# calclavia/tal-asrd

Measured on AMD Instinct MI355X. Metric: audio frames/sec (16 kHz, 10 ms hop) end-to-end log-mel -> TDS encoder -> diarization head, higher is better.
Workload: dtype f32 (dense layers: 3 x f16 MFMA hi/lo split, f32 accumulate); 1 GPU; 1 x 3600 s 16 kHz clip per GPU, each a whole-episode B=1 call (BASELINE.json configs[2]; SDModel path of tal/baseline/reconcile.py:76-85: log-mel -> TDS 80-800-1120-1440 -> 128-d feat + argmax over 6008 speakers); weights=synthetic deterministic, audio_resident_in_hbm=True

## Files before the change

tal_asrd_amd/csrc/gemm_common.h:

```cpp
#pragma once
#include "common.h"

namespace tal {

constexpr int BK = 32;

template <int MODE, int NSUB>
__device__ __forceinline__ void gemm_epilogue(const GemmArgs& g, const f32x16 (&acc)[NSUB], float* lds, float* Y,
                                              const float* bias, const float* res, int64_t m0, int n0, int lane,
                                              int w, int wm, int wn) {
    const int64_t M = g.M;
    const int N = g.N;
    const int colb = lane & 31;
    const int rowb = 4 * (lane >> 5);
    const float alpha = g.alpha;
    const f32x4 zero4 = {0.f, 0.f, 0.f, 0.f};
    float amax = 0.f;
    constexpr int CW = 32 * NSUB;
    if (MODE == 4) {
        float bcol[NSUB];
#pragma unroll
        for (int j = 0; j < NSUB; ++j) {
            const int col = n0 + (wn * NSUB + j) * 32 + colb;
            bcol[j] = (bias && col < N) ? bias[col] : 0.f;
        }
        const int pcol = (n0 / CW) + wn;
#pragma unroll
        for (int e = 0; e < 16; ++e) {
            float best = -INFINITY;
            int bi = 0x7fffffff;
#pragma unroll
            for (int j = 0; j < NSUB; ++j) {
                const int col = n0 + (wn * NSUB + j) * 32 + colb;
                const float v = acc[j][e] + bcol[j];
                if (col < N && v > best) {
                    best = v;
                    bi = col;
                }
            }
#pragma unroll
            for (int off = 16; off > 0; off >>= 1) {
                const float ov = __shfl_xor(best, off, 64);
                const int oi = __shfl_xor(bi, off, 64);
                if (ov > best || (ov == best && oi < bi)) {
                    best = ov;
                    bi = oi;
                }
            }
            const int64_t row = m0 + wm * 32 + rowb + (e & 3) + 8 * (e >> 2);
            if (colb == 0 && row < M) {
                g.part_val[row * g.part_ld + pcol] = best;
                g.part_idx[row * g.part_ld + pcol] = bi;
            }
        }
        return;
    }
    const bool vec_ok = (g.ldy % 4 == 0) && (MODE != 2 || g.ldres % 4 == 0) &&
                        ((reinterpret_cast<uintptr_t>(Y) & 15) == 0) &&
                        (MODE != 2 || (reinterpret_cast<uintptr_t>(res) & 15) == 0);
    if (vec_ok) {
        float* stage = lds + w * (16 * CW);
        const int n_base = n0 + wn * CW;
        const bool cols_full = n_base + CW <= N;
        const bool buf_ok = g.ldy < (1 << 21) && (MODE != 2 || g.ldres < (1 << 21));
        auto uptr = [](const float* p) {
            const uint64_t v = reinterpret_cast<uint64_t>(p);
            const uint32_t lo = __builtin_amdgcn_readfirstlane((uint32_t)v), hi = __builtin_amdgcn_readfirstlane((uint32_t)(v >> 32));
            return reinterpret_cast<void*>(((uint64_t)hi << 32) | lo);
        };
        __amdgpu_buffer_rsrc_t rs_y[2], rs_res[2];
#pragma unroll
        for (int half = 0; half < 2; ++half) {
            const int64_t row0 = m0 + wm * 32 + half * 16;
            const int rows_valid = (int)(M - row0 < 0 ? 0 : (M - row0 > 16 ? 16 : M - row0));
            const int ext_y = rows_valid > 0 ? (int)(((rows_valid - 1) * g.ldy + CW) * 4) : 0;
            const int ext_r = rows_valid > 0 && MODE == 2 ? (int)(((rows_valid - 1) * g.ldres + CW) * 4) : 0;
            rs_y[half] = __builtin_amdgcn_make_buffer_rsrc(uptr(Y + row0 * g.ldy + n_base), 0, __builtin_amdgcn_readfirstlane(ext_y), 0x00020000);
            rs_res[half] = __builtin_amdgcn_make_buffer_rsrc(uptr(MODE == 2 ? res + row0 * g.ldres + n_base : Y), 0,
                                                             __builtin_amdgcn_readfirstlane(ext_r), 0x00020000);
        }
        __amdgpu_buffer_rsrc_t rs_bias = __builtin_amdgcn_make_buffer_rsrc(uptr(bias ? bias + n_base : Y), 0, CW * 4, 0x00020000);
#pragma unroll
        for (int half = 0; half < 2; ++half) {
#pragma unroll
            for (int j = 0; j < NSUB; ++j)
#pragma unroll
                for (int e8 = 0; e8 < 8; ++e8) {
                    const int e = half * 8 + e8;
                    const int r = rowb + (e8 & 3) + 8 * (e8 >> 2);
                    stage[r * CW + j * 32 + colb] = acc[j][e];
                }
            if (cols_full && buf_ok) {
                typedef unsigned u32x4 __attribute__((ext_vector_type(4)));
                int r = lane / (CW / 4), c4 = lane - r * (CW / 4);
                int offy[2 * NSUB], offr[2 * NSUB], offb[2 * NSUB], ldsv[2 * NSUB];
                f32x4 rv[2 * NSUB], bv[2 * NSUB];
#pragma unroll
                for (int t = 0; t < 2 * NSUB; ++t) {
                    offy[t] = (r * (int)g.ldy + c4 * 4) * 4;
                    offr[t] = (r * (int)g.ldres + c4 * 4) * 4;
                    offb[t] = c4 * 16;
                    ldsv[t] = r * CW + c4 * 4;
                    c4 += 64 - CW / 4;
                    r += 1;
                    if (c4 >= CW / 4) {
                        c4 -= CW / 4;
                        r += 1;
                    }
                }
                typedef unsigned u32x2r __attribute__((ext_vector_type(2)));
                u32x2r rh[2 * NSUB], rl[2 * NSUB];
#pragma unroll
                for (int t = 0; t < 2 * NSUB; ++t) {
                    if (MODE == 2 && g.res_split) {
                        const int cw = offb[t] >> 2;
                        const int so = offr[t] - offb[t] + (cw >> 5) * 128 + (cw & 31) * 2;
                        rh[t] = __builtin_amdgcn_raw_buffer_load_b64(rs_res[half], so, 0, 0);
                        rl[t] = __builtin_amdgcn_raw_buffer_load_b64(rs_res[half], so + 64, 0, 0);
                    } else if (MODE == 2)
                        rv[t] = __builtin_bit_cast(f32x4, __builtin_amdgcn_raw_buffer_load_b128(rs_res[half], offr[t], 0, 0));
                    bv[t] = bias ? __builtin_bit_cast(f32x4, __builtin_amdgcn_raw_buffer_load_b128(rs_bias, offb[t], 0, 0)) : zero4;
                }
#pragma unroll
                for (int t = 0; t < 2 * NSUB; ++t) {
// ... 38 lines not shown
                if (g.out_split && half == 1) note_range(amax, g.range_flag);
                continue;
            }
#pragma unroll
            for (int t = 0; t < 2 * NSUB; ++t) {
                const int i = lane + 64 * t;
                const int r = i / (CW / 4);
                const int c = (i - r * (CW / 4)) * 4;
                const int64_t row = m0 + wm * 32 + half * 16 + r;
                const int col = n_base + c;
                if (row < M && col < N) {
                    f32x4 v = *reinterpret_cast<const f32x4*>(&stage[r * CW + c]);
                    if (col + 3 < N) {
                        if (bias) v += *reinterpret_cast<const f32x4*>(bias + col);
                        if (MODE == 1) {
                            v.x = fmaxf(v.x, 0.f); v.y = fmaxf(v.y, 0.f); v.z = fmaxf(v.z, 0.f); v.w = fmaxf(v.w, 0.f);
                        }
                        if (MODE == 2) v = *reinterpret_cast<const f32x4*>(res + row * g.ldres + col) + alpha * v;
                        if (MODE == 3 && (g.scale_cols == 0 || col < g.scale_cols)) v = alpha * v;
                        *reinterpret_cast<f32x4*>(Y + row * g.ldy + col) = v;
                    } else {
                        for (int q = 0; q < 4 && col + q < N; ++q) {
                            float x = v[q] + (bias ? bias[col + q] : 0.f);
                            if (MODE == 1) x = fmaxf(x, 0.f);
                            if (MODE == 2) x = res[row * g.ldres + col + q] + alpha * x;
                            if (MODE == 3 && (g.scale_cols == 0 || col + q < g.scale_cols)) x = alpha * x;
                            Y[row * g.ldy + col + q] = x;
                        }
                    }
                }
            }
        }
    } else {
#pragma unroll
        for (int j = 0; j < NSUB; ++j) {
            const int col = n0 + (wn * NSUB + j) * 32 + colb;
            if (col >= N) continue;
            const float bv = bias ? bias[col] : 0.f;
#pragma unroll
            for (int e = 0; e < 16; ++e) {
                const int64_t row = m0 + wm * 32 + rowb + (e & 3) + 8 * (e >> 2);
                if (row < M) {
                    float v = acc[j][e] + bv;
                    if (MODE == 1) v = fmaxf(v, 0.f);
                    if (MODE == 2) v = res[row * g.ldres + col] + alpha * v;
                    if (MODE == 3 && (g.scale_cols == 0 || col < g.scale_cols)) v = alpha * v;
                    Y[row * g.ldy + col] = v;
                }
            }
        }
    }
}

template <int MODE, int NSUB>
__device__ __forceinline__ void gemm_epilogue_split(const GemmArgs& g, const f32x16 (&acc)[NSUB], float* lds, float* Y,
                                                    const float* res, int64_t m0, int n0, int lane, int w) {
    static_assert(MODE == 1 || MODE == 2, "relu or residual");
    constexpr int CW = 32 * NSUB;
    typedef unsigned u32x2 __attribute__((ext_vector_type(2)));
    typedef float f32x2 __attribute__((ext_vector_type(2)));
    const int64_t M = g.M;
    const int colb = lane & 31, rowb = 4 * (lane >> 5);
    float* stage = lds + w * (16 * CW);
    auto uptr = [](const float* p) {
        const uint64_t v = reinterpret_cast<uint64_t>(p);
        const uint32_t lo = __builtin_amdgcn_readfirstlane((uint32_t)v), hi = __builtin_amdgcn_readfirstlane((uint32_t)(v >> 32));
        return reinterpret_cast<void*>(((uint64_t)hi << 32) | lo);
    };
    const int lr = lane >> 3, lp = lane & 7;
    const int ldy4 = (int)g.ldy * 4, ldr4 = (int)g.ldres * 4;
    const int vy0 = lr * ldy4 + lp * 8, vy1 = vy0 + 8 * ldy4;
    const int vr0 = lr * ldr4 + lp * 8, vr1 = vr0 + 8 * ldr4;
    const float* sp = stage + lr * CW + lp * 4;
    const float alpha = g.alpha;
    const f32x2 al2 = {alpha, alpha}, s11 = {1.0f / 2048.0f, 1.0f / 2048.0f};
    float amax = 0.f;
#pragma unroll
    for (int half = 0; half < 2; ++half) {
        const int64_t row0 = m0 + w * 32 + half * 16;
        const int rows_valid = (int)(M - row0 < 0 ? 0 : (M - row0 > 16 ? 16 : M - row0));
        const int ext_y = rows_valid > 0 ? (rows_valid - 1) * ldy4 + CW * 4 : 0;
        const int ext_r = rows_valid > 0 && MODE == 2 ? (rows_valid - 1) * ldr4 + CW * 4 : 0;
        __amdgpu_buffer_rsrc_t rs_y = __builtin_amdgcn_make_buffer_rsrc(uptr(Y + row0 * g.ldy + n0), 0, __builtin_amdgcn_readfirstlane(ext_y), 0x00020000);
        __amdgpu_buffer_rsrc_t rs_r = __builtin_amdgcn_make_buffer_rsrc(uptr(MODE == 2 ? res + row0 * g.ldres + n0 : Y), 0,
                                                                      __builtin_amdgcn_readfirstlane(ext_r), 0x00020000);
        u32x2 rh[2 * NSUB], rl[2 * NSUB];
        if (MODE == 2) {
#pragma unroll
            for (int t = 0; t < 2 * NSUB; ++t) {
                const int rg = t / NSUB, b = t % NSUB;
                rh[t] = __builtin_amdgcn_raw_buffer_load_b64(rs_r, (rg ? vr1 : vr0) + b * 128, 0, 0);
                rl[t] = __builtin_amdgcn_raw_buffer_load_b64(rs_r, (rg ? vr1 : vr0) + b * 128 + 64, 0, 0);
            }
        }
#pragma unroll
        for (int j = 0; j < NSUB; ++j)
#pragma unroll
            for (int e8 = 0; e8 < 8; ++e8) {
                const int r = rowb + (e8 & 3) + 8 * (e8 >> 2);
                stage[r * CW + j * 32 + colb] = acc[j][half * 8 + e8];
            }
        f32x4 sv[2 * NSUB];
#pragma unroll
        for (int t = 0; t < 2 * NSUB; ++t) sv[t] = *reinterpret_cast<const f32x4*>(sp + (t / NSUB) * 8 * CW + (t % NSUB) * 32);
#pragma unroll
        for (int t = 0; t < 2 * NSUB; ++t) {
            const int rg = t / NSUB, b = t % NSUB;
            f32x2 va = {sv[t][0], sv[t][1]}, vb = {sv[t][2], sv[t][3]};
            if (MODE == 1) {
                va = __builtin_elementwise_max(va, f32x2{0.f, 0.f});
                vb = __builtin_elementwise_max(vb, f32x2{0.f, 0.f});
            } else {
                const f16x4 h4 = __builtin_bit_cast(f16x4, rh[t]), l4 = __builtin_bit_cast(f16x4, rl[t]);
                const f32x2 ha = {(float)h4[0], (float)h4[1]}, hb = {(float)h4[2], (float)h4[3]};
                const f32x2 la = {(float)l4[0], (float)l4[1]}, lb = {(float)l4[2], (float)l4[3]};
                va = al2 * va + (la * s11 + ha);
                vb = al2 * vb + (lb * s11 + hb);
            }
            amax = __builtin_fmaxf(amax, __builtin_fmaxf(__builtin_fabsf(va[0]), __builtin_fabsf(va[1])));
            amax = __builtin_fmaxf(amax, __builtin_fmaxf(__builtin_fabsf(vb[0]), __builtin_fabsf(vb[1])));
            f16x2p h01, l01, h23, l23;
            split_f16x3_pair(va[0], va[1], h01, l01);
            split_f16x3_pair(vb[0], vb[1], h23, l23);
            const f16x4 hi = {h01[0], h01[1], h23[0], h23[1]}, lo = {l01[0], l01[1], l23[0], l23[1]};
            __builtin_amdgcn_raw_buffer_store_b64(__builtin_bit_cast(u32x2, hi), rs_y, (rg ? vy1 : vy0) + b * 128, 0, 0);
            __builtin_amdgcn_raw_buffer_store_b64(__builtin_bit_cast(u32x2, lo), rs_y, (rg ? vy1 : vy0) + b * 128 + 64, 0, 0);
        }
    }
    note_range(amax, g.range_flag);
}

__device__ __forceinline__ unsigned logical_tile_of(unsigned nb, unsigned bid) {
    const unsigned xcd = bid & 7u, q = nb >> 3, r = nb & 7u;
    return (xcd < r ? xcd * (q + 1) : r * (q + 1) + (xcd - r) * q) + (bid >> 3);
// ... 5 lines not shown
```

tal_asrd_amd/csrc/gemm_f32.hip:

```cpp
#include "gemm_common.h"

namespace tal {

template <int MODE, int NSUB, bool SPLITK, int STAGE, bool F16X3 = false, int EPI = 0>
__global__ __launch_bounds__(256, F16X3 ? 2 : 1) void gemm_glds_kernel(const GemmArgs g) {
    __builtin_amdgcn_s_setprio(3);
    constexpr int BM = 128, BN = 32 * NSUB;
    constexpr int ROWS = BM + BN;
    constexpr int CHUNKS = ROWS / 8;
    constexpr int PER_WAVE = CHUNKS / 4;
    __shared__ __attribute__((aligned(16))) float lds[2 * ROWS * 32];

    const bool is_slice = SPLITK && blockIdx.x >= (unsigned)g.tile_base;
    const unsigned sbid = blockIdx.x - (unsigned)g.tile_base;
    const int slice = is_slice ? (int)(sbid / (unsigned)g.tail_tiles) : 0;
    const unsigned logical = is_slice ? (unsigned)g.tile_base + sbid % (unsigned)g.tail_tiles
                                      : (SPLITK ? logical_tile_of((unsigned)g.tile_base, blockIdx.x) : logical_tile());
    const unsigned tile_m = g.tiles_n == 1 ? logical : __umulhi(logical, g.tiles_n_magic);
    const int64_t m0 = (int64_t)tile_m * BM;
    const int n0 = (int)(logical - tile_m * (unsigned)g.tiles_n) * BN;
    const int64_t M = g.M;
    const int N = g.N, K = g.K;
    const int z1 = EPI ? 0 : (int)blockIdx.y / g.nb2, z2 = EPI ? 0 : (int)blockIdx.y % g.nb2;
    const float* A = g.A + z1 * g.a_s1 + z2 * g.a_s2;
// ... 18 lines not shown
        if (t < 4)
            src[t] = A + (m0 + min(row, a_rows)) * g.lda + srccol;
        else
            src[t] = W + (int64_t)(n0 + min(row - BM, b_rows)) * g.ldw + srccol;
    }
    auto uniform_ptr = [](const float* p) {
        const uint64_t v = reinterpret_cast<uint64_t>(p);
        const uint32_t lo = __builtin_amdgcn_readfirstlane((uint32_t)v), hi = __builtin_amdgcn_readfirstlane((uint32_t)(v >> 32));
        return reinterpret_cast<void*>(((uint64_t)hi << 32) | lo);
    };
    __amdgpu_buffer_rsrc_t rsrc_a = __builtin_amdgcn_make_buffer_rsrc(uniform_ptr(A + m0 * g.lda), 0, 0x7fffffff, 0x00020000);
    __amdgpu_buffer_rsrc_t rsrc_w = __builtin_amdgcn_make_buffer_rsrc(uniform_ptr(W + (int64_t)n0 * g.ldw), 0, 0x7fffffff, 0x00020000);
    int voff[PER_WAVE];
#pragma unroll
    for (int t = 0; t < PER_WAVE; ++t) {
        const int row = 8 * (w + 4 * t) + sub;
        voff[t] = t < 4 ? (int)((min(row, a_rows) * g.lda + srccol) * 4) : (int)((min(row - BM, b_rows) * g.ldw + srccol) * 4);
    }
    auto issue = [&](int kt, int buf) {
#pragma unroll
        for (int t = 0; t < PER_WAVE; ++t) {
            float* dst = lds + buf * (ROWS * 32) + (w + 4 * t) * 256;
            if (STAGE == 2) {
#if defined(__HIP_DEVICE_COMPILE__)
                __builtin_amdgcn_raw_ptr_buffer_load_lds(t < 4 ? rsrc_a : rsrc_w, (__attribute__((address_space(3))) void*)dst, 16,
                                                         voff[t], kt * (BK * 4), 0, 0);
#endif
            } else
                __builtin_amdgcn_global_load_lds((const __attribute__((address_space(1))) void*)(src[t] + kt * BK),
                                                 (__attribute__((address_space(3))) void*)dst, 16, 0, 0);
        }
    };

    f32x16 acc[NSUB];
    f32x16 accx[F16X3 ? NSUB : 1];
#pragma unroll
    for (int j = 0; j < NSUB; ++j) {
        const float b0 = (EPI && bias && !is_slice) ? bias[n0 + j * 32 + (lane & 31)] : 0.f;
#pragma unroll
        for (int e = 0; e < 16; ++e) acc[j][e] = b0;
    }
#pragma unroll
    for (int j = 0; j < (F16X3 ? NSUB : 1); ++j)
#pragma unroll
        for (int e = 0; e < 16; ++e) accx[j][e] = 0.f;

    const int frow = lane & 31;
    const int fsw = (frow >> 1) & 7;
    const int fhalf = lane >> 5;
    const int nk_all = K / BK;
    const int kt0 = is_slice ? (int)((int64_t)slice * nk_all / g.split) : 0;
    const int nk = is_slice ? (int)((int64_t)(slice + 1) * nk_all / g.split) : nk_all;
    issue(kt0, kt0 & 1);
    __builtin_amdgcn_s_setprio(0);
    __builtin_assume(kt0 < nk);
    for (int kt = kt0; kt < nk; ++kt) {
        asm volatile("s_waitcnt vmcnt(0)" ::: "memory");
        __syncthreads();
        if (kt + 1 < nk) issue(kt + 1, (kt + 1) & 1);
        const float* As = lds + (kt & 1) * (ROWS * 32) + (wm * 32 + frow) * 32;
        const float* Bs = lds + (kt & 1) * (ROWS * 32) + (BM + frow) * 32;
        if (F16X3) {
            f16x8 ahi[2], alo[2], bhi[3], blo[3];
            auto slh = [&](int gk) { return ((2 * gk + fhalf) ^ fsw) * 4; };
            auto sll = [&](int gk) { return ((4 + 2 * gk + fhalf) ^ fsw) * 4; };
            auto read_b = [&](int q, int slot) {
                const int gk = q / NSUB, j = q % NSUB;
                bhi[slot] = *reinterpret_cast<const f16x8*>(Bs + j * 32 * 32 + slh(gk));
                blo[slot] = *reinterpret_cast<const f16x8*>(Bs + j * 32 * 32 + sll(gk));
            };
            ahi[0] = *reinterpret_cast<const f16x8*>(As + slh(0));
            alo[0] = *reinterpret_cast<const f16x8*>(As + sll(0));
            read_b(0, 0);
            read_b(1, 1);
#pragma unroll
            for (int q = 0; q < 2 * NSUB; ++q) {
                const int gk = q / NSUB, j = q % NSUB;
                if (q + 2 < 2 * NSUB) read_b(q + 2, (q + 2) % 3);
                if (q == NSUB - 2) {
                    ahi[1] = *reinterpret_cast<const f16x8*>(As + slh(1));
                    alo[1] = *reinterpret_cast<const f16x8*>(As + sll(1));
                }
                __builtin_amdgcn_sched_barrier(0);
                acc[j] = __builtin_amdgcn_mfma_f32_32x32x16_f16(ahi[gk], bhi[q % 3], acc[j], 0, 0, 0);
                accx[F16X3 ? j : 0] = __builtin_amdgcn_mfma_f32_32x32x16_f16(ahi[gk], blo[q % 3], accx[F16X3 ? j : 0], 0, 0, 0);
                accx[F16X3 ? j : 0] = __builtin_amdgcn_mfma_f32_32x32x16_f16(alo[gk], bhi[q % 3], accx[F16X3 ? j : 0], 0, 0, 0);
                __builtin_amdgcn_sched_barrier(0);
            }
            continue;
        }
        f32x4 fa[2], fb[2][NSUB];
        fa[0] = *reinterpret_cast<const f32x4*>(As + ((fhalf) ^ fsw) * 4);
#pragma unroll
        for (int j = 0; j < NSUB; ++j) fb[0][j] = *reinterpret_cast<const f32x4*>(Bs + j * 32 * 32 + ((fhalf) ^ fsw) * 4);
#pragma unroll
        for (int kk = 0; kk < BK / 8; ++kk) {
            const int cur = kk & 1, nxt = cur ^ 1;
            if (kk + 1 < BK / 8) {
                const int sl = ((2 * (kk + 1) + fhalf) ^ fsw) * 4;
                fa[nxt] = *reinterpret_cast<const f32x4*>(As + sl);
#pragma unroll
                for (int j = 0; j < NSUB; ++j) fb[nxt][j] = *reinterpret_cast<const f32x4*>(Bs + j * 32 * 32 + sl);
            }
#pragma unroll
            for (int j = 0; j < NSUB; ++j) {
                acc[j] = __builtin_amdgcn_mfma_f32_32x32x2f32(fa[cur].x, fb[cur][j].x, acc[j], 0, 0, 0);
                acc[j] = __builtin_amdgcn_mfma_f32_32x32x2f32(fa[cur].y, fb[cur][j].y, acc[j], 0, 0, 0);
                acc[j] = __builtin_amdgcn_mfma_f32_32x32x2f32(fa[cur].z, fb[cur][j].z, acc[j], 0, 0, 0);
                acc[j] = __builtin_amdgcn_mfma_f32_32x32x2f32(fa[cur].w, fb[cur][j].w, acc[j], 0, 0, 0);
            }
        }
    }
    asm volatile("s_waitcnt vmcnt(0)" ::: "memory");
    __syncthreads();
    __builtin_amdgcn_s_setprio(3);
    if (F16X3) {
        typedef float f32x2 __attribute__((ext_vector_type(2)));
        const f32x2 s11 = {1.0f / 2048.0f, 1.0f / 2048.0f};
#pragma unroll
        for (int j = 0; j < NSUB; ++j)
#pragma unroll
            for (int e = 0; e < 16; e += 2) {
                const f32x2 x2 = {accx[F16X3 ? j : 0][e], accx[F16X3 ? j : 0][e + 1]}, a2 = {acc[j][e], acc[j][e + 1]};
                const f32x2 o2 = __builtin_elementwise_fma(x2, s11, a2);
                acc[j][e] = o2[0];
                acc[j][e + 1] = o2[1];
            }
    }
    if (is_slice) {
        GemmArgs gp = g;
        gp.M = m0 + BM;
        gp.N = n0 + BN;
        gp.ldy = BN;
        gp.out_split = 0;
        float* tile_ws = g.splitk_ws + ((size_t)(logical - g.tile_base) * g.split + slice) * (BM * BN);
        gemm_epilogue<0, NSUB>(gp, acc, lds, tile_ws - (m0 * BN + n0), nullptr, nullptr, m0, n0, lane, w, wm, wn);
    } else {
        if constexpr (EPI != 0) gemm_epilogue_split<MODE, NSUB>(g, acc, lds, Y, res, m0, n0, lane, w);
        else gemm_epilogue<MODE, NSUB>(g, acc, lds, Y, bias, res, m0, n0, lane, w, wm, wn);
    }
}

template <int MODE, int WAVES_M, int NSUB, int BKT>
__global__ __launch_bounds__(256) void gemm_nt_f32_kernel(const GemmArgs g) {
    constexpr int WAVES_N = 4 / WAVES_M;
    constexpr int BM = 32 * WAVES_M;
    constexpr int BN = 32 * NSUB * WAVES_N;
    constexpr int LDS_LD = BKT + 4;
    constexpr int C4 = BKT / 4;
    constexpr int RPP = 256 / C4;
    constexpr int A_LOADS = BM / RPP;
    constexpr int B_LOADS = BN / RPP;
    __shared__ __attribute__((aligned(16))) float lds[(BM + BN) * LDS_LD];
    float* As = lds;
    float* Bs = lds + BM * LDS_LD;

    const unsigned logical = logical_tile();
    const int64_t m0 = (int64_t)(logical / (unsigned)g.tiles_n) * BM;
    const int n0 = (int)(logical % (unsigned)g.tiles_n) * BN;
    const int64_t M = g.M;
    const int N = g.N, K = g.K;

    const int z1 = (int)blockIdx.y / g.nb2, z2 = (int)blockIdx.y % g.nb2;
    const float* A = g.A + z1 * g.a_s1 + z2 * g.a_s2;
    const float* W = g.W + z1 * g.w_s1 + z2 * g.w_s2;
    float* Y = g.Y + z1 * g.y_s1 + z2 * g.y_s2;
    const float* bias = g.bias ? g.bias + z2 * g.bias_s2 : nullptr;
    const float* res = g.res ? g.res + z1 * g.r_s1 + z2 * g.r_s2 : nullptr;

    const int tid = threadIdx.x;
    const int lane = tid & 63;
    const int w = wave_id();
// ... 554 lines not shown
```

tal_asrd_amd/csrc/gemm_w64.hip:

```cpp
#include <type_traits>

#include "gemm_common.h"

namespace tal {

namespace {

typedef unsigned u32x4w __attribute__((ext_vector_type(4)));

constexpr int W_BM = 256, W_NSUB = 5, W_BN = 32 * W_NSUB, W_ROWS = W_BM + W_BN, W_NBUF = 3;
constexpr int W_CHUNKS = W_ROWS / 8, W_PER_WAVE = W_CHUNKS / 4, W_AT = W_BM / 8 / 4;
constexpr int W_BUF_FLOATS = W_ROWS * 32;
static_assert(W_CHUNKS % 4 == 0, "chunks divide over the waves");

constexpr int dma_piece(int q, int slot) { return (slot < 2 && q < 6) ? 2 * q + slot : (q == 6 && slot == 0) ? 12 : -1; }

__device__ __forceinline__ void mfma_vgpr(f32x16& c, const f16x8& a, const f16x8& b) {
    asm volatile("v_mfma_f32_32x32x16_f16 %0, %1, %2, %0" : "+v"(c) : "v"(a), "v"(b));
}
#define W64_MFMA(c, a, b, in_vgpr) do { if (in_vgpr) mfma_vgpr(c, a, b); else c = __builtin_amdgcn_mfma_f32_32x32x16_f16(a, b, c, 0, 0, 0); } while (0)

struct Frags {
    f16x8 ahi[2][2], alo[2][2];
    f16x8 bhi[5], blo[5];
};

}

template <int MODE, bool SPLITK, int EPI>
__global__ __launch_bounds__(256, 1) void gemm_w64_kernel(const GemmArgs g) {
    constexpr int NSUB = W_NSUB, BM = W_BM, BN = W_BN, PER_WAVE = W_PER_WAVE, A_T = W_AT, BUF_FLOATS = W_BUF_FLOATS;
    __shared__ __attribute__((aligned(16))) float lds[W_NBUF * W_BUF_FLOATS];

    if (g.stagger_ticks > 0 && blockIdx.x < (unsigned)g.stagger_blocks && (blockIdx.x & 1u)) {
        const unsigned long long t0 = wall_clock64();
        while (wall_clock64() - t0 < (unsigned long long)g.stagger_ticks) __builtin_amdgcn_s_sleep(64);
    }
    const bool is_slice = SPLITK && blockIdx.x >= (unsigned)g.tile_base;
    const unsigned sbid = blockIdx.x - (unsigned)g.tile_base;
    const int slice = is_slice ? (int)(sbid / (unsigned)g.tail_tiles) : 0;
    const unsigned logical = is_slice ? (unsigned)g.tile_base + sbid % (unsigned)g.tail_tiles
                                      : (SPLITK ? logical_tile_of((unsigned)g.tile_base, blockIdx.x) : logical_tile());
    const unsigned tile_m = g.tiles_n == 1 ? logical : __umulhi(logical, g.tiles_n_magic);
    const int64_t m0 = (int64_t)tile_m * BM;
    const int n0 = (int)(logical - tile_m * (unsigned)g.tiles_n) * BN;
    const int64_t M = g.M;
    const int N = g.N, K = g.K;
    const float* A = g.A;
    const float* W = g.W;
    const int tid = threadIdx.x, lane = tid & 63;
    const int w = wave_id();

    const int sub = lane >> 3, srccol = ((lane & 7) ^ (((w & 1) * 4 + (lane >> 4)) & 7)) * 4;
    const int a_rows = (int)((M - m0) < BM ? (M - m0) : BM) - 1;
    const int b_rows = ((N - n0) < BN ? (N - n0) : BN) - 1;
    auto make_rsrc = [](const float* p) {
        const uint64_t v = reinterpret_cast<uint64_t>(p);
        u32x4w r;
        r[0] = __builtin_amdgcn_readfirstlane((uint32_t)v);
        r[1] = __builtin_amdgcn_readfirstlane((uint32_t)(v >> 32));
        r[2] = 0x7fffffffu;
        r[3] = 0x00020000u;
        return r;
    };
    const u32x4w rs_a = make_rsrc(A + m0 * g.lda), rs_w = make_rsrc(W + (int64_t)n0 * g.ldw);
    const unsigned lds_base = __builtin_amdgcn_readfirstlane((unsigned)(size_t)(__attribute__((address_space(3))) float*)lds) + (unsigned)w * 1024u;
    int voff[PER_WAVE];
#pragma unroll
    for (int t = 0; t < PER_WAVE; ++t) {
        const int row = 8 * (w + 4 * t) + sub;
        voff[t] = t < A_T ? (int)((min(row, a_rows) * g.lda + srccol) * 4) : (int)((min(row - BM, b_rows) * g.ldw + srccol) * 4);
    }
    auto dma = [&](int t, unsigned nrec, int bufoff, int kofs) {
        const unsigned dst = lds_base + (unsigned)(bufoff * 4 + t * 4096);
        u32x4w rs = t < A_T ? rs_a : rs_w;
        rs[2] = nrec;
        asm volatile("s_mov_b32 m0, %0\n\ts_nop 0\n\tbuffer_load_dwordx4 %1, %2, %3 offen lds" ::"s"(dst), "v"(voff[t]), "s"(rs), "s"(kofs) : "memory");
    };

    f32x16 hh[2][NSUB], xx[2][NSUB];
#pragma unroll
    for (int j = 0; j < NSUB; ++j) {
        const float b0 = (EPI && g.bias && !is_slice) ? g.bias[n0 + j * 32 + (lane & 31)] : 0.f;
#pragma unroll
        for (int b = 0; b < 2; ++b)
#pragma unroll
            for (int e = 0; e < 16; ++e) {
                hh[b][j][e] = b0;
                xx[b][j][e] = 0.f;
            }
    }

    const int frow = lane & 31, fsw = (frow >> 1) & 7, fhalf = lane >> 5, fc = fhalf ^ fsw;
    const int a_lane = (w * 64 + frow) * 32, b_lane = (BM + frow) * 32;
    auto slot = [&](int x) { return (x ^ fc) * 4; };
    Frags f;
    auto read_a = [&](int gk, int bufoff) {
#pragma unroll
        for (int b = 0; b < 2; ++b) {
            f.ahi[gk][b] = *reinterpret_cast<const f16x8*>(lds + bufoff + a_lane + b * 32 * 32 + slot(2 * gk));
            f.alo[gk][b] = *reinterpret_cast<const f16x8*>(lds + bufoff + a_lane + b * 32 * 32 + slot(4 + 2 * gk));
        }
    };
    auto rb = [&](int q, int bufoff) {
        const int gk = q / NSUB, j = q % NSUB;
        f.bhi[j] = *reinterpret_cast<const f16x8*>(lds + bufoff + b_lane + j * 32 * 32 + slot(2 * gk));
        f.blo[j] = *reinterpret_cast<const f16x8*>(lds + bufoff + b_lane + j * 32 * 32 + slot(4 + 2 * gk));
    };

    const int nk_all = K / BK;
    const int kt0 = is_slice ? (int)((int64_t)slice * nk_all / g.split) : 0;
    const int kt1 = is_slice ? (int)((int64_t)(slice + 1) * nk_all / g.split) : nk_all;
    constexpr unsigned NREC = 0x7fffffffu;
#pragma unroll
    for (int t = 0; t < PER_WAVE; ++t) dma(t, NREC, 0, kt0 * (BK * 4));
    {
        const unsigned nrec = kt0 + 1 < kt1 ? NREC : 0u;
#pragma unroll
        for (int t = 0; t < PER_WAVE; ++t) dma(t, nrec, BUF_FLOATS, (kt0 + 1) * (BK * 4));
    }
    asm volatile("s_waitcnt vmcnt(%0)" ::"n"(PER_WAVE) : "memory");
    __builtin_amdgcn_s_barrier();
    read_a(0, 0);
    rb(0, 0);
    rb(1, 0);
    auto step = [&](auto bufc, int kt) {
        constexpr int cur = decltype(bufc)::value * BUF_FLOATS, nxt = ((decltype(bufc)::value + 1) % 3) * BUF_FLOATS,
                      fil = ((decltype(bufc)::value + 2) % 3) * BUF_FLOATS;
        const int kofs = (kt + 2) * (BK * 4);
        const unsigned nrec = kt + 2 < kt1 ? NREC : 0u;
#pragma unroll
        for (int q = 0; q < 2 * NSUB; ++q) {
            const int gk = q / NSUB, j = q % NSUB;
            if (q == 8) {
                asm volatile("s_waitcnt vmcnt(%0)" ::"n"(PER_WAVE) : "memory");
                __builtin_amdgcn_s_barrier();
            }
            if (q + 2 < 2 * NSUB) rb(q + 2, cur);
            else rb(q + 2 - 2 * NSUB, nxt);
            if (q == 8) read_a(0, nxt);
            if (q == 2) read_a(1, cur);
            __builtin_amdgcn_sched_barrier(0);
            const bool vg = j >= 3, vx0 = j >= 4;
            W64_MFMA(hh[0][j], f.ahi[gk][0], f.bhi[j], false);
            W64_MFMA(hh[1][j], f.ahi[gk][1], f.bhi[j], vg);
            if (dma_piece(q, 0) >= 0) { __builtin_amdgcn_sched_barrier(0); dma(dma_piece(q, 0), nrec, fil, kofs); __builtin_amdgcn_sched_barrier(0); }
            W64_MFMA(xx[0][j], f.ahi[gk][0], f.blo[j], vx0);
            W64_MFMA(xx[1][j], f.ahi[gk][1], f.blo[j], vg);
            if (dma_piece(q, 1) >= 0) { __builtin_amdgcn_sched_barrier(0); dma(dma_piece(q, 1), nrec, fil, kofs); __builtin_amdgcn_sched_barrier(0); }
            W64_MFMA(xx[0][j], f.alo[gk][0], f.bhi[j], vx0);
            W64_MFMA(xx[1][j], f.alo[gk][1], f.bhi[j], vg);
            if (dma_piece(q, 2) >= 0) { __builtin_amdgcn_sched_barrier(0); dma(dma_piece(q, 2), nrec, fil, kofs); }
            __builtin_amdgcn_sched_barrier(0);
        }
    };
    int kt = kt0;
    for (; kt + 3 <= kt1; kt += 3) {
        step(std::integral_constant<int, 0>(), kt);
        step(std::integral_constant<int, 1>(), kt + 1);
        step(std::integral_constant<int, 2>(), kt + 2);
    }
    if (kt < kt1) step(std::integral_constant<int, 0>(), kt);
    if (kt + 1 < kt1) step(std::integral_constant<int, 1>(), kt + 1);
    asm volatile("s_waitcnt vmcnt(0)\n\ts_nop 15\n\ts_nop 15" ::: "memory");
    __syncthreads();

    typedef float f32x2 __attribute__((ext_vector_type(2)));
    const f32x2 s11 = {1.0f / 2048.0f, 1.0f / 2048.0f};
    auto finish = [&](auto bc) {
        constexpr int b = decltype(bc)::value;
        f32x16 acc[NSUB];
#pragma unroll
        for (int j = 0; j < NSUB; ++j)
#pragma unroll
            for (int e = 0; e < 16; e += 2) {
                const f32x2 x2 = {xx[b][j][e], xx[b][j][e + 1]}, a2 = {hh[b][j][e], hh[b][j][e + 1]};
                const f32x2 o2 = __builtin_elementwise_fma(x2, s11, a2);
                acc[j][e] = o2[0];
                acc[j][e + 1] = o2[1];
            }
        const int64_t m0e = m0 + 32 * w + 32 * b;
        if (b == 1) __builtin_amdgcn_wave_barrier();
        if (is_slice) {
            GemmArgs gp = g;
            gp.M = m0 + BM;
            gp.N = n0 + BN;
            gp.ldy = BN;
            gp.out_split = 0;
            float* tile_ws = g.splitk_ws + ((size_t)(logical - g.tile_base) * g.split + slice) * (BM * BN);
            gemm_epilogue<0, NSUB>(gp, acc, lds, tile_ws - (m0 * BN + n0), nullptr, nullptr, m0e, n0, lane, w, w, 0);
        } else {
            if constexpr (EPI != 0) gemm_epilogue_split<MODE, NSUB>(g, acc, lds, g.Y, g.res, m0e, n0, lane, w);
            else gemm_epilogue<MODE, NSUB>(g, acc, lds, g.Y, g.bias, g.res, m0e, n0, lane, w, w, 0);
        }
    };
    finish(std::integral_constant<int, 0>());
    finish(std::integral_constant<int, 1>());
}

template <int MODE, bool SPLITK>
static void launch_w64_mode(const GemmArgs& g, dim3 grid, hipStream_t s) {
    if constexpr (MODE == 1 || MODE == 2) {
        const bool y_ok = g.ldy % 4 == 0 && g.ldy < (1 << 21) && (reinterpret_cast<uintptr_t>(g.Y) & 15) == 0 && g.N % W_BN == 0;
        const bool r_ok = MODE != 2 || (g.res_split && g.ldres % 4 == 0 && g.ldres < (1 << 21) && (reinterpret_cast<uintptr_t>(g.res) & 15) == 0);
        if (g.out_split && g.range_flag && y_ok && r_ok) {
            hipLaunchKernelGGL((gemm_w64_kernel<MODE, SPLITK, 1>), grid, dim3(256), 0, s, g);
            return;
        }
    }
    hipLaunchKernelGGL((gemm_w64_kernel<MODE, SPLITK, 0>), grid, dim3(256), 0, s, g);
}

void launch_gemm_w64(const GemmArgs& g0, int mode, bool splitk, dim3 grid, hipStream_t s) {
    GemmArgs g = g0;
    const int pct = opt(OPT_GEMM_W64_STAGGER);
    if (pct > 0 && grid.x >= 2u * (unsigned)device_cus()) {
        const double tile_us = 1.39 * (g.K / 32) + 12.0;
        g.stagger_ticks = (int)(tile_us * pct);
        g.stagger_blocks = device_cus();
    }
    if (splitk) {
        switch (mode) {
            case 0: launch_w64_mode<0, true>(g, grid, s); break;
            case 1: launch_w64_mode<1, true>(g, grid, s); break;
            case 2: launch_w64_mode<2, true>(g, grid, s); break;
            default: launch_w64_mode<3, true>(g, grid, s); break;
// ... 13 lines not shown
```

Before: 21.01 million frames/s.

## Switch f16x3 GEMM paths from 32x32x16 to 16x16x32 MFMA tiles

Replaces the 32x32x16 f16 MFMA in the hi/lo split GEMM kernels (gemm_f32 and the w64 kernel) with 16x16x32 MFMA over 16-row/16-col sub-blocks. Accumulators, LDS fragment addressing and swizzle, and the epilogue staging are reworked for the 16x16 accumulator layout. The w64 kernel also double-buffers its A fragments across k-steps and unrolls the k-loop by six. The aim is a better MFMA issue rate and latency hiding per k-step, at the cost of more MFMA instructions, more LDS fragment reads and higher register pressure from the doubled A fragment sets.

Result: faster. 21.67 million frames/s (median of 6 runs) (+3.1%).

```diff
diff --git a/tal_asrd_amd/csrc/gemm_common.h b/tal_asrd_amd/csrc/gemm_common.h
--- a/tal_asrd_amd/csrc/gemm_common.h
+++ b/tal_asrd_amd/csrc/gemm_common.h
@@ -5,10 +5,38 @@
 
 constexpr int BK = 32;
 
-template <int MODE, int NSUB>
-__device__ __forceinline__ void gemm_epilogue(const GemmArgs& g, const f32x16 (&acc)[NSUB], float* lds, float* Y,
+template <int NSUB, bool L16>
+struct GemmAcc { typedef f32x16 type[NSUB]; };
+template <int NSUB>
+struct GemmAcc<NSUB, true> { typedef f32x4 type[2][2 * NSUB]; };
+
+template <int NSUB>
+__device__ __forceinline__ void gemm_stage_half(float* stage, const f32x16 (&acc)[NSUB], int half, int lane) {
+    constexpr int CW = 32 * NSUB;
+    const int colb = lane & 31, rowb = 4 * (lane >> 5);
+#pragma unroll
+    for (int j = 0; j < NSUB; ++j)
+#pragma unroll
+        for (int e8 = 0; e8 < 8; ++e8) {
+            const int r = rowb + (e8 & 3) + 8 * (e8 >> 2);
+            stage[r * CW + j * 32 + colb] = acc[j][half * 8 + e8];
+        }
+}
+template <int NSUB>
+__device__ __forceinline__ void gemm_stage_half(float* stage, const f32x4 (&acc)[2][2 * NSUB], int half, int lane) {
+    constexpr int CW = 32 * NSUB;
+    const int colb = lane & 15, rowb = 4 * (lane >> 4);
+#pragma unroll
+    for (int j = 0; j < 2 * NSUB; ++j)
+#pragma unroll
+        for (int e = 0; e < 4; ++e) stage[(rowb + e) * CW + j * 16 + colb] = acc[half][j][e];
+}
+
+template <int MODE, int NSUB, bool L16 = false>
+__device__ __forceinline__ void gemm_epilogue(const GemmArgs& g, const typename GemmAcc<NSUB, L16>::type& acc, float* lds, float* Y,
                                               const float* bias, const float* res, int64_t m0, int n0, int lane,
                                               int w, int wm, int wn) {
+    static_assert(!(L16 && MODE == 4), "the fused arg-max reads the 32x32 layout");
     const int64_t M = g.M;
     const int N = g.N;
     const int colb = lane & 31;
@@ -17,7 +45,7 @@
     const f32x4 zero4 = {0.f, 0.f, 0.f, 0.f};
     float amax = 0.f;
     constexpr int CW = 32 * NSUB;
-    if (MODE == 4) {
+    if constexpr (MODE == 4) {
         float bcol[NSUB];
 #pragma unroll
         for (int j = 0; j < NSUB; ++j) {
@@ -82,14 +110,7 @@
         __amdgpu_buffer_rsrc_t rs_bias = __builtin_amdgcn_make_buffer_rsrc(uptr(bias ? bias + n_base : Y), 0, CW * 4, 0x00020000);
 #pragma unroll
         for (int half = 0; half < 2; ++half) {
-#pragma unroll
-            for (int j = 0; j < NSUB; ++j)
-#pragma unroll
-                for (int e8 = 0; e8 < 8; ++e8) {
-                    const int e = half * 8 + e8;
-                    const int r = rowb + (e8 & 3) + 8 * (e8 >> 2);
-                    stage[r * CW + j * 32 + colb] = acc[j][e];
-                }
+            gemm_stage_half<NSUB>(stage, acc, half, lane);
             if (cols_full && buf_ok) {
                 typedef unsigned u32x4 __attribute__((ext_vector_type(4)));
                 int r = lane / (CW / 4), c4 = lane - r * (CW / 4);
@@ -194,35 +215,47 @@
             }
         }
     } else {
-#pragma unroll
-        for (int j = 0; j < NSUB; ++j) {
-            const int col = n0 + (wn * NSUB + j) * 32 + colb;
-            if (col >= N) continue;
-            const float bv = bias ? bias[col] : 0.f;
-#pragma unroll
-            for (int e = 0; e < 16; ++e) {
-                const int64_t row = m0 + wm * 32 + rowb + (e & 3) + 8 * (e >> 2);
-                if (row < M) {
-                    float v = acc[j][e] + bv;
-                    if (MODE == 1) v = fmaxf(v, 0.f);
-                    if (MODE == 2) v = res[row * g.ldres + col] + alpha * v;
-                    if (MODE == 3 && (g.scale_cols == 0 || col < g.scale_cols)) v = alpha * v;
-                    Y[row * g.ldy + col] = v;
-                }
+        auto finish_one = [&](int64_t row, int col, float bv, float a) {
+            if (row < M) {
+                float v = a + bv;
+                if (MODE == 1) v = fmaxf(v, 0.f);
+                if (MODE == 2) v = res[row * g.ldres + col] + alpha * v;
+                if (MODE == 3 && (g.scale_cols == 0 || col < g.scale_cols)) v = alpha * v;
+                Y[row * g.ldy + col] = v;
+            }
+        };
+        if constexpr (L16) {
+#pragma unroll
+            for (int j = 0; j < 2 * NSUB; ++j) {
+                const int col = n0 + wn * CW + j * 16 + (lane & 15);
+                if (col >= N) continue;
+                const float bv = bias ? bias[col] : 0.f;
+#pragma unroll
+                for (int i = 0; i < 2; ++i)
+#pragma unroll
+                    for (int e = 0; e < 4; ++e) finish_one(m0 + wm * 32 + 16 * i + 4 * (lane >> 4) + e, col, bv, acc[i][j][e]);
+            }
+        } else {
+#pragma unroll
+            for (int j = 0; j < NSUB; ++j) {
+                const int col = n0 + (wn * NSUB + j) * 32 + colb;
+                if (col >= N) continue;
+                const float bv = bias ? bias[col] : 0.f;
+#pragma unroll
+                for (int e = 0; e < 16; ++e) finish_one(m0 + wm * 32 + rowb + (e & 3) + 8 * (e >> 2), col, bv, acc[j][e]);
             }
         }
     }
 }
 
-template <int MODE, int NSUB>
-__device__ __forceinline__ void gemm_epilogue_split(const GemmArgs& g, const f32x16 (&acc)[NSUB], float* lds, float* Y,
+template <int MODE, int NSUB, bool L16 = false>
+__device__ __forceinline__ void gemm_epilogue_split(const GemmArgs& g, const typename GemmAcc<NSUB, L16>::type& acc, float* lds, float* Y,
                                                     const float* res, int64_t m0, int n0, int lane, int w) {
     static_assert(MODE == 1 || MODE == 2, "relu or residual");
     constexpr int CW = 32 * NSUB;
     typedef unsigned u32x2 __attribute__((ext_vector_type(2)));
     typedef float f32x2 __attribute__((ext_vector_type(2)));
     const int64_t M = g.M;
-    const int colb = lane & 31, rowb = 4 * (lane >> 5);
     float* stage = lds + w * (16 * CW);
     auto uptr = [](const float* p) {
         const uint64_t v = reinterpret_cast<uint64_t>(p);
@@ -255,13 +288,7 @@
                 rl[t] = __builtin_amdgcn_raw_buffer_load_b64(rs_r, (rg ? vr1 : vr0) + b * 128 + 64, 0, 0);
             }
         }
-#pragma unroll
-        for (int j = 0; j < NSUB; ++j)
-#pragma unroll
-            for (int e8 = 0; e8 < 8; ++e8) {
-                const int r = rowb + (e8 & 3) + 8 * (e8 >> 2);
-                stage[r * CW + j * 32 + colb] = acc[j][half * 8 + e8];
-            }
+        gemm_stage_half<NSUB>(stage, acc, half, lane);
         f32x4 sv[2 * NSUB];
 #pragma unroll
         for (int t = 0; t < 2 * NSUB; ++t) sv[t] = *reinterpret_cast<const f32x4*>(sp + (t / NSUB) * 8 * CW + (t % NSUB) * 32);
diff --git a/tal_asrd_amd/csrc/gemm_f32.hip b/tal_asrd_amd/csrc/gemm_f32.hip
--- a/tal_asrd_amd/csrc/gemm_f32.hip
+++ b/tal_asrd_amd/csrc/gemm_f32.hip
@@ -74,18 +74,27 @@
         }
     };
 
-    f32x16 acc[NSUB];
-    f32x16 accx[F16X3 ? NSUB : 1];
-#pragma unroll
-    for (int j = 0; j < NSUB; ++j) {
-        const float b0 = (EPI && bias && !is_slice) ? bias[n0 + j * 32 + (lane & 31)] : 0.f;
-#pragma unroll
-        for (int e = 0; e < 16; ++e) acc[j][e] = b0;
-    }
-#pragma unroll
-    for (int j = 0; j < (F16X3 ? NSUB : 1); ++j)
-#pragma unroll
-        for (int e = 0; e < 16; ++e) accx[j][e] = 0.f;
+    constexpr int CB = 2 * NSUB;
+    f32x16 acc[F16X3 ? 1 : NSUB];
+    f32x4 acc16[F16X3 ? 2 : 1][F16X3 ? CB : 1], accx[F16X3 ? 2 : 1][F16X3 ? CB : 1];
+    if (F16X3) {
+#pragma unroll
+        for (int j = 0; j < CB; ++j) {
+            const float b0 = (EPI && bias && !is_slice) ? bias[n0 + j * 16 + (lane & 15)] : 0.f;
+#pragma unroll
+            for (int i = 0; i < 2; ++i)
+#pragma unroll
+                for (int e = 0; e < 4; ++e) {
+                    acc16[F16X3 ? i : 0][F16X3 ? j : 0][e] = b0;
+                    accx[F16X3 ? i : 0][F16X3 ? j : 0][e] = 0.f;
+                }
+        }
+    } else {
+#pragma unroll
+        for (int j = 0; j < NSUB; ++j)
+#pragma unroll
+            for (int e = 0; e < 16; ++e) acc[F16X3 ? 0 : j][e] = 0.f;
+    }
 
     const int frow = lane & 31;
     const int fsw = (frow >> 1) & 7;
@@ -103,30 +112,32 @@
         const float* As = lds + (kt & 1) * (ROWS * 32) + (wm * 32 + frow) * 32;
         const float* Bs = lds + (kt & 1) * (ROWS * 32) + (BM + frow) * 32;
         if (F16X3) {
+            const int r16 = lane & 15, q16 = lane >> 4, sw16 = (r16 >> 1) & 7;
+            const int slh = (q16 ^ sw16) * 4, sll = ((4 + q16) ^ sw16) * 4;
+            const float* As16 = lds + (kt & 1) * (ROWS * 32) + (wm * 32 + r16) * 32;
+            const float* Bs16 = lds + (kt & 1) * (ROWS * 32) + (BM + r16) * 32;
             f16x8 ahi[2], alo[2], bhi[3], blo[3];
-            auto slh = [&](int gk) { return ((2 * gk + fhalf) ^ fsw) * 4; };
-            auto sll = [&](int gk) { return ((4 + 2 * gk + fhalf) ^ fsw) * 4; };
-            auto read_b = [&](int q, int slot) {
-                const int gk = q / NSUB, j = q % NSUB;
-                bhi[slot] = *reinterpret_cast<const f16x8*>(Bs + j * 32 * 32 + slh(gk));
-                blo[slot] = *reinterpret_cast<const f16x8*>(Bs + j * 32 * 32 + sll(gk));
+            auto read_b = [&](int j, int slot) {
+                bhi[slot] = *reinterpret_cast<const f16x8*>(Bs16 + j * 16 * 32 + slh);
+                blo[slot] = *reinterpret_cast<const f16x8*>(Bs16 + j * 16 * 32 + sll);
             };
-            ahi[0] = *reinterpret_cast<const f16x8*>(As + slh(0));
-            alo[0] = *reinterpret_cast<const f16x8*>(As + sll(0));
+            ahi[0] = *reinterpret_cast<const f16x8*>(As16 + slh);
+            ahi[1] = *reinterpret_cast<const f16x8*>(As16 + 16 * 32 + slh);
             read_b(0, 0);
+            alo[0] = *reinterpret_cast<const f16x8*>(As16 + sll);
+            alo[1] = *reinterpret_cast<const f16x8*>(As16 + 16 * 32 + sll);
             read_b(1, 1);
 #pragma unroll
-            for (int q = 0; q < 2 * NSUB; ++q) {
-                const int gk = q / NSUB, j = q % NSUB;
-                if (q + 2 < 2 * NSUB) read_b(q + 2, (q + 2) % 3);
-                if (q == NSUB - 2) {
-                    ahi[1] = *reinterpret_cast<const f16x8*>(As + slh(1));
-                    alo[1] = *reinterpret_cast<const f16x8*>(As + sll(1));
-                }
+            for (int j = 0; j < CB; ++j) {
+                constexpr int Z = F16X3 ? 1 : 0;
+                if (j + 2 < CB) read_b(j + 2, (j + 2) % 3);
                 __builtin_amdgcn_sched_barrier(0);
-                acc[j] = __builtin_amdgcn_mfma_f32_32x32x16_f16(ahi[gk], bhi[q % 3], acc[j], 0, 0, 0);
-                accx[F16X3 ? j : 0] = __builtin_amdgcn_mfma_f32_32x32x16_f16(ahi[gk], blo[q % 3], accx[F16X3 ? j : 0], 0, 0, 0);
-                accx[F16X3 ? j : 0] = __builtin_amdgcn_mfma_f32_32x32x16_f16(alo[gk], bhi[q % 3], accx[F16X3 ? j : 0], 0, 0, 0);
+                acc16[0][Z * j] = __builtin_amdgcn_mfma_f32_16x16x32_f16(ahi[0], bhi[j % 3], acc16[0][Z * j], 0, 0, 0);
+                acc16[Z][Z * j] = __builtin_amdgcn_mfma_f32_16x16x32_f16(ahi[1], bhi[j % 3], acc16[Z][Z * j], 0, 0, 0);
+                accx[0][Z * j] = __builtin_amdgcn_mfma_f32_16x16x32_f16(ahi[0], blo[j % 3], accx[0][Z * j], 0, 0, 0);
+                accx[Z][Z * j] = __builtin_amdgcn_mfma_f32_16x16x32_f16(ahi[1], blo[j % 3], accx[Z][Z * j], 0, 0, 0);
+                accx[0][Z * j] = __builtin_amdgcn_mfma_f32_16x16x32_f16(alo[0], bhi[j % 3], accx[0][Z * j], 0, 0, 0);
+                accx[Z][Z * j] = __builtin_amdgcn_mfma_f32_16x16x32_f16(alo[1], bhi[j % 3], accx[Z][Z * j], 0, 0, 0);
                 __builtin_amdgcn_sched_barrier(0);
             }
             continue;
@@ -146,28 +157,31 @@
             }
 #pragma unroll
             for (int j = 0; j < NSUB; ++j) {
-                acc[j] = __builtin_amdgcn_mfma_f32_32x32x2f32(fa[cur].x, fb[cur][j].x, acc[j], 0, 0, 0);
-                acc[j] = __builtin_amdgcn_mfma_f32_32x32x2f32(fa[cur].y, fb[cur][j].y, acc[j], 0, 0, 0);
-                acc[j] = __builtin_amdgcn_mfma_f32_32x32x2f32(fa[cur].z, fb[cur][j].z, acc[j], 0, 0, 0);
-                acc[j] = __builtin_amdgcn_mfma_f32_32x32x2f32(fa[cur].w, fb[cur][j].w, acc[j], 0, 0, 0);
+                constexpr int Z = F16X3 ? 0 : 1;
+                acc[Z * j] = __builtin_amdgcn_mfma_f32_32x32x2f32(fa[cur].x, fb[cur][j].x, acc[Z * j], 0, 0, 0);
+                acc[Z * j] = __builtin_amdgcn_mfma_f32_32x32x2f32(fa[cur].y, fb[cur][j].y, acc[Z * j], 0, 0, 0);
+                acc[Z * j] = __builtin_amdgcn_mfma_f32_32x32x2f32(fa[cur].z, fb[cur][j].z, acc[Z * j], 0, 0, 0);
+                acc[Z * j] = __builtin_amdgcn_mfma_f32_32x32x2f32(fa[cur].w, fb[cur][j].w, acc[Z * j], 0, 0, 0);
             }
         }
     }
     asm volatile("s_waitcnt vmcnt(0)" ::: "memory");
     __syncthreads();
     __builtin_amdgcn_s_setprio(3);
-    if (F16X3) {
+    if constexpr (F16X3) {
         typedef float f32x2 __attribute__((ext_vector_type(2)));
         const f32x2 s11 = {1.0f / 2048.0f, 1.0f / 2048.0f};
 #pragma unroll
-        for (int j = 0; j < NSUB; ++j)
-#pragma unroll
-            for (int e = 0; e < 16; e += 2) {
-                const f32x2 x2 = {accx[F16X3 ? j : 0][e], accx[F16X3 ? j : 0][e + 1]}, a2 = {acc[j][e], acc[j][e + 1]};
-                const f32x2 o2 = __builtin_elementwise_fma(x2, s11, a2);
-                acc[j][e] = o2[0];
-                acc[j][e + 1] = o2[1];
-            }
+        for (int i = 0; i < 2; ++i)
+#pragma unroll
+            for (int j = 0; j < CB; ++j)
+#pragma unroll
+                for (int e = 0; e < 4; e += 2) {
+                    const f32x2 x2 = {accx[i][j][e], accx[i][j][e + 1]}, a2 = {acc16[i][j][e], acc16[i][j][e + 1]};
+                    const f32x2 o2 = __builtin_elementwise_fma(x2, s11, a2);
+                    acc16[i][j][e] = o2[0];
+                    acc16[i][j][e + 1] = o2[1];
+                }
     }
     if (is_slice) {
         GemmArgs gp = g;
@@ -176,10 +190,13 @@
         gp.ldy = BN;
         gp.out_split = 0;
         float* tile_ws = g.splitk_ws + ((size_t)(logical - g.tile_base) * g.split + slice) * (BM * BN);
-        gemm_epilogue<0, NSUB>(gp, acc, lds, tile_ws - (m0 * BN + n0), nullptr, nullptr, m0, n0, lane, w, wm, wn);
+        if constexpr (F16X3) gemm_epilogue<0, NSUB, true>(gp, acc16, lds, tile_ws - (m0 * BN + n0), nullptr, nullptr, m0, n0, lane, w, wm, wn);
+        else gemm_epilogue<0, NSUB>(gp, acc, lds, tile_ws - (m0 * BN + n0), nullptr, nullptr, m0, n0, lane, w, wm, wn);
+    } else if constexpr (F16X3) {
+        if constexpr (EPI != 0) gemm_epilogue_split<MODE, NSUB, true>(g, acc16, lds, Y, res, m0, n0, lane, w);
+        else gemm_epilogue<MODE, NSUB, true>(g, acc16, lds, Y, bias, res, m0, n0, lane, w, wm, wn);
     } else {
-        if constexpr (EPI != 0) gemm_epilogue_split<MODE, NSUB>(g, acc, lds, Y, res, m0, n0, lane, w);
-        else gemm_epilogue<MODE, NSUB>(g, acc, lds, Y, bias, res, m0, n0, lane, w, wm, wn);
+        gemm_epilogue<MODE, NSUB>(g, acc, lds, Y, bias, res, m0, n0, lane, w, wm, wn);
     }
 }
 
diff --git a/tal_asrd_amd/csrc/gemm_w64.hip b/tal_asrd_amd/csrc/gemm_w64.hip
--- a/tal_asrd_amd/csrc/gemm_w64.hip
+++ b/tal_asrd_amd/csrc/gemm_w64.hip
@@ -15,13 +15,18 @@
 
 constexpr int dma_piece(int q, int slot) { return (slot < 2 && q < 6) ? 2 * q + slot : (q == 6 && slot == 0) ? 12 : -1; }
 
-__device__ __forceinline__ void mfma_vgpr(f32x16& c, const f16x8& a, const f16x8& b) {
-    asm volatile("v_mfma_f32_32x32x16_f16 %0, %1, %2, %0" : "+v"(c) : "v"(a), "v"(b));
-}
-#define W64_MFMA(c, a, b, in_vgpr) do { if (in_vgpr) mfma_vgpr(c, a, b); else c = __builtin_amdgcn_mfma_f32_32x32x16_f16(a, b, c, 0, 0, 0); } while (0)
+constexpr int W_RB = 4, W_CB = 2 * W_NSUB;
+
+__device__ __forceinline__ void mfma_vgpr(f32x4& c, const f16x8& a, const f16x8& b) {
+    asm volatile("v_mfma_f32_16x16x32_f16 %0, %1, %2, %0" : "+v"(c) : "v"(a), "v"(b));
+}
+__device__ __forceinline__ void mfma_agpr(f32x4& c, const f16x8& a, const f16x8& b) {
+    asm volatile("v_mfma_f32_16x16x32_f16 %0, %1, %2, %0" : "+a"(c) : "v"(a), "v"(b));
+}
+#define W64_MFMA(c, a, b, in_vgpr) do { if (in_vgpr) mfma_vgpr(c, a, b); else mfma_agpr(c, a, b); } while (0)
 
 struct Frags {
-    f16x8 ahi[2][2], alo[2][2];
+    f16x8 ahi[2][W_RB], alo[2][W_RB];
     f16x8 bhi[5], blo[5];
 };
 
@@ -29,7 +34,7 @@
 
 template <int MODE, bool SPLITK, int EPI>
 __global__ __launch_bounds__(256, 1) void gemm_w64_kernel(const GemmArgs g) {
-    constexpr int NSUB = W_NSUB, BM = W_BM, BN = W_BN, PER_WAVE = W_PER_WAVE, A_T = W_AT, BUF_FLOATS = W_BUF_FLOATS;
+    constexpr int NSUB = W_NSUB, RB = W_RB, CB = W_CB, BM = W_BM, BN = W_BN, PER_WAVE = W_PER_WAVE, A_T = W_AT, BUF_FLOATS = W_BUF_FLOATS;
     __shared__ __attribute__((aligned(16))) float lds[W_NBUF * W_BUF_FLOATS];
 
     if (g.stagger_ticks > 0 && blockIdx.x < (unsigned)g.stagger_blocks && (blockIdx.x & 1u)) {
@@ -78,34 +83,34 @@
         asm volatile("s_mov_b32 m0, %0\n\ts_nop 0\n\tbuffer_load_dwordx4 %1, %2, %3 offen lds" ::"s"(dst), "v"(voff[t]), "s"(rs), "s"(kofs) : "memory");
     };
 
-    f32x16 hh[2][NSUB], xx[2][NSUB];
-#pragma unroll
-    for (int j = 0; j < NSUB; ++j) {
-        const float b0 = (EPI && g.bias && !is_slice) ? g.bias[n0 + j * 32 + (lane & 31)] : 0.f;
-#pragma unroll
-        for (int b = 0; b < 2; ++b)
-#pragma unroll
-            for (int e = 0; e < 16; ++e) {
-                hh[b][j][e] = b0;
-                xx[b][j][e] = 0.f;
+    f32x4 hh[RB][CB], xx[RB][CB];
+#pragma unroll
+    for (int j = 0; j < CB; ++j) {
+        const float b0 = (EPI && g.bias && !is_slice) ? g.bias[n0 + j * 16 + (lane & 15)] : 0.f;
+#pragma unroll
+        for (int i = 0; i < RB; ++i)
+#pragma unroll
+            for (int e = 0; e < 4; ++e) {
+                hh[i][j][e] = b0;
+                xx[i][j][e] = 0.f;
             }
     }
 
-    const int frow = lane & 31, fsw = (frow >> 1) & 7, fhalf = lane >> 5, fc = fhalf ^ fsw;
+    const int frow = lane & 15, fsw = (frow >> 1) & 7, fq = lane >> 4;
     const int a_lane = (w * 64 + frow) * 32, b_lane = (BM + frow) * 32;
-    auto slot = [&](int x) { return (x ^ fc) * 4; };
+    const int sh = (fq ^ fsw) * 4, sl = ((4 + fq) ^ fsw) * 4;
     Frags f;
-    auto read_a = [&](int gk, int bufoff) {
-#pragma unroll
-        for (int b = 0; b < 2; ++b) {
-            f.ahi[gk][b] = *reinterpret_cast<const f16x8*>(lds + bufoff + a_lane + b * 32 * 32 + slot(2 * gk));
-            f.alo[gk][b] = *reinterpret_cast<const f16x8*>(lds + bufoff + a_lane + b * 32 * 32 + slot(4 + 2 * gk));
-        }
-    };
-    auto rb = [&](int q, int bufoff) {
-        const int gk = q / NSUB, j = q % NSUB;
-        f.bhi[j] = *reinterpret_cast<const f16x8*>(lds + bufoff + b_lane + j * 32 * 32 + slot(2 * gk));
-        f.blo[j] = *reinterpret_cast<const f16x8*>(lds + bufoff + b_lane + j * 32 * 32 + slot(4 + 2 * gk));
+    auto read_ahi = [&](int set, int bufoff) {
+#pragma unroll
+        for (int i = 0; i < RB; ++i) f.ahi[set][i] = *reinterpret_cast<const f16x8*>(lds + bufoff + a_lane + i * 16 * 32 + sh);
+    };
+    auto read_alo = [&](int set, int bufoff) {
+#pragma unroll
+        for (int i = 0; i < RB; ++i) f.alo[set][i] = *reinterpret_cast<const f16x8*>(lds + bufoff + a_lane + i * 16 * 32 + sl);
+    };
+    auto rb = [&](int j, int bufoff) {
+        f.bhi[j % 5] = *reinterpret_cast<const f16x8*>(lds + bufoff + b_lane + j * 16 * 32 + sh);
+        f.blo[j % 5] = *reinterpret_cast<const f16x8*>(lds + bufoff + b_lane + j * 16 * 32 + sl);
     };
 
     const int nk_all = K / BK;
@@ -121,47 +126,56 @@
     }
     asm volatile("s_waitcnt vmcnt(%0)" ::"n"(PER_WAVE) : "memory");
     __builtin_amdgcn_s_barrier();
-    read_a(0, 0);
+    read_ahi(0, 0);
     rb(0, 0);
     rb(1, 0);
-    auto step = [&](auto bufc, int kt) {
+    read_alo(0, 0);
+    auto step = [&](auto bufc, auto setc, int kt) {
         constexpr int cur = decltype(bufc)::value * BUF_FLOATS, nxt = ((decltype(bufc)::value + 1) % 3) * BUF_FLOATS,
-                      fil = ((decltype(bufc)::value + 2) % 3) * BUF_FLOATS;
+                      fil = ((decltype(bufc)::value + 2) % 3) * BUF_FLOATS, set = decltype(setc)::value;
         const int kofs = (kt + 2) * (BK * 4);
         const unsigned nrec = kt + 2 < kt1 ? NREC : 0u;
 #pragma unroll
-        for (int q = 0; q < 2 * NSUB; ++q) {
-            const int gk = q / NSUB, j = q % NSUB;
+        for (int q = 0; q < CB; ++q) {
+            const int s = q % 5;
             if (q == 8) {
                 asm volatile("s_waitcnt vmcnt(%0)" ::"n"(PER_WAVE) : "memory");
                 __builtin_amdgcn_s_barrier();
             }
-            if (q + 2 < 2 * NSUB) rb(q + 2, cur);
-            else rb(q + 2 - 2 * NSUB, nxt);
-            if (q == 8) read_a(0, nxt);
-            if (q == 2) read_a(1, cur);
+            if (q + 2 < CB) rb(q + 2, cur);
+            else rb(q + 2 - CB, nxt);
+            if (q == 8) read_ahi(set ^ 1, nxt);
+            if (q == 9) read_alo(set ^ 1, nxt);
             __builtin_amdgcn_sched_barrier(0);
-            const bool vg = j >= 3, vx0 = j >= 4;
-            W64_MFMA(hh[0][j], f.ahi[gk][0], f.bhi[j], false);
-            W64_MFMA(hh[1][j], f.ahi[gk][1], f.bhi[j], vg);
+#pragma unroll
+            for (int i = 0; i < RB; ++i) W64_MFMA(hh[i][q], f.ahi[set][i], f.bhi[s], i == RB - 1);
             if (dma_piece(q, 0) >= 0) { __builtin_amdgcn_sched_barrier(0); dma(dma_piece(q, 0), nrec, fil, kofs); __builtin_amdgcn_sched_barrier(0); }
-            W64_MFMA(xx[0][j], f.ahi[gk][0], f.blo[j], vx0);
-            W64_MFMA(xx[1][j], f.ahi[gk][1], f.blo[j], vg);
+#pragma unroll
+            for (int i = 0; i < RB; ++i) W64_MFMA(xx[i][q], f.ahi[set][i], f.blo[s], i == RB - 1);
             if (dma_piece(q, 1) >= 0) { __builtin_amdgcn_sched_barrier(0); dma(dma_piece(q, 1), nrec, fil, kofs); __builtin_amdgcn_sched_barrier(0); }
-            W64_MFMA(xx[0][j], f.alo[gk][0], f.bhi[j], vx0);
-            W64_MFMA(xx[1][j], f.alo[gk][1], f.bhi[j], vg);
+#pragma unroll
+            for (int i = 0; i < RB; ++i) W64_MFMA(xx[i][q], f.alo[set][i], f.bhi[s], i == RB - 1);
             if (dma_piece(q, 2) >= 0) { __builtin_amdgcn_sched_barrier(0); dma(dma_piece(q, 2), nrec, fil, kofs); }
             __builtin_amdgcn_sched_barrier(0);
         }
     };
+    using I0 = std::integral_constant<int, 0>;
+    using I1 = std::integral_constant<int, 1>;
+    using I2 = std::integral_constant<int, 2>;
     int kt = kt0;
-    for (; kt + 3 <= kt1; kt += 3) {
-        step(std::integral_constant<int, 0>(), kt);
-        step(std::integral_constant<int, 1>(), kt + 1);
-        step(std::integral_constant<int, 2>(), kt + 2);
-    }
-    if (kt < kt1) step(std::integral_constant<int, 0>(), kt);
-    if (kt + 1 < kt1) step(std::integral_constant<int, 1>(), kt + 1);
+    for (; kt + 6 <= kt1; kt += 6) {
+        step(I0(), I0(), kt);
+        step(I1(), I1(), kt + 1);
+        step(I2(), I0(), kt + 2);
+        step(I0(), I1(), kt + 3);
+        step(I1(), I0(), kt + 4);
+        step(I2(), I1(), kt + 5);
+    }
+    if (kt < kt1) step(I0(), I0(), kt);
+    if (kt + 1 < kt1) step(I1(), I1(), kt + 1);
+    if (kt + 2 < kt1) step(I2(), I0(), kt + 2);
+    if (kt + 3 < kt1) step(I0(), I1(), kt + 3);
+    if (kt + 4 < kt1) step(I1(), I0(), kt + 4);
     asm volatile("s_waitcnt vmcnt(0)\n\ts_nop 15\n\ts_nop 15" ::: "memory");
     __syncthreads();
 
@@ -169,16 +183,18 @@
     const f32x2 s11 = {1.0f / 2048.0f, 1.0f / 2048.0f};
     auto finish = [&](auto bc) {
         constexpr int b = decltype(bc)::value;
-        f32x16 acc[NSUB];
-#pragma unroll
-        for (int j = 0; j < NSUB; ++j)
-#pragma unroll
-            for (int e = 0; e < 16; e += 2) {
-                const f32x2 x2 = {xx[b][j][e], xx[b][j][e + 1]}, a2 = {hh[b][j][e], hh[b][j][e + 1]};
-                const f32x2 o2 = __builtin_elementwise_fma(x2, s11, a2);
-                acc[j][e] = o2[0];
-                acc[j][e + 1] = o2[1];
-            }
+        f32x4 acc[2][CB];
+#pragma unroll
+        for (int i = 0; i < 2; ++i)
+#pragma unroll
+            for (int j = 0; j < CB; ++j)
+#pragma unroll
+                for (int e = 0; e < 4; e += 2) {
+                    const f32x2 x2 = {xx[2 * b + i][j][e], xx[2 * b + i][j][e + 1]}, a2 = {hh[2 * b + i][j][e], hh[2 * b + i][j][e + 1]};
+                    const f32x2 o2 = __builtin_elementwise_fma(x2, s11, a2);
+                    acc[i][j][e] = o2[0];
+                    acc[i][j][e + 1] = o2[1];
+                }
         const int64_t m0e = m0 + 32 * w + 32 * b;
         if (b == 1) __builtin_amdgcn_wave_barrier();
         if (is_slice) {
@@ -188,10 +204,10 @@
             gp.ldy = BN;
             gp.out_split = 0;
             float* tile_ws = g.splitk_ws + ((size_t)(logical - g.tile_base) * g.split + slice) * (BM * BN);
-            gemm_epilogue<0, NSUB>(gp, acc, lds, tile_ws - (m0 * BN + n0), nullptr, nullptr, m0e, n0, lane, w, w, 0);
+            gemm_epilogue<0, NSUB, true>(gp, acc, lds, tile_ws - (m0 * BN + n0), nullptr, nullptr, m0e, n0, lane, w, w, 0);
         } else {
-            if constexpr (EPI != 0) gemm_epilogue_split<MODE, NSUB>(g, acc, lds, g.Y, g.res, m0e, n0, lane, w);
-            else gemm_epilogue<MODE, NSUB>(g, acc, lds, g.Y, g.bias, g.res, m0e, n0, lane, w, w, 0);
+            if constexpr (EPI != 0) gemm_epilogue_split<MODE, NSUB, true>(g, acc, lds, g.Y, g.res, m0e, n0, lane, w);
+            else gemm_epilogue<MODE, NSUB, true>(g, acc, lds, g.Y, g.bias, g.res, m0e, n0, lane, w, w, 0);
         }
     };
     finish(std::integral_constant<int, 0>());
```
